# yoshitomo-matsubara/hnd-ghnd-object-detectors

Measured on AMD Instinct MI355X. Metric: distill-step images/sec at 3x800x1333, GHND Faster R-CNN b3ch, higher is better.
Workload: dtype f32

## Files before the change

hnd_ghnd_object_detectors_amd/_lib.py:

```python
import collections
import ctypes as C
import os
import re

_HERE = os.path.dirname(os.path.abspath(__file__))
LIB_PATH = os.environ.get('HND_LIB_PATH') or os.path.join(_HERE, 'libhnd_hip.so')
INCLUDE_DIR = os.path.join(os.path.dirname(_HERE), 'include')


class HndLibraryError(RuntimeError):
    pass


Header = collections.namedtuple('Header', 'defines enums structs functions')
_SCALARS = {'int': C.c_int, 'int32_t': C.c_int32, 'int64_t': C.c_int64, 'size_t': C.c_size_t, 'float': C.c_float,
            'double': C.c_double}
_POINTEES = ('void', 'float', 'double', 'int64_t', 'uint8_t', 'uint16_t', 'unsigned char')
_DIRECTIVE = re.compile(r'#\s*(include\s*<\w+\.h>|ifndef\s+\w+|define\s+\w+)$')
_TYPEDEF = re.compile(r'typedef\s+(enum|struct)\s+(\w+)\s*\{([^{}]*)\}\s*(\w+)\s*;')
_PROTOTYPE = re.compile(r'([^;{}()]+)\(([^;{}()]*)\)\s*;')
_DECLARATION = re.compile(r'\s*(?:const\s+)?(unsigned\s+char|\w+)(\s*\*+\s*|\s+)(\w+)\s*(\[\d*\])?\s*$')
_ENUMERATOR = re.compile(r'\s*(\w+)\s*=\s*(-?\d+)\s*$')
_SPACE = re.compile(r'\s*')

# ... 77 lines not shown
def _read(fname):
    path = os.path.join(INCLUDE_DIR, fname)
    if not os.path.isfile(path):
        raise HndLibraryError('C header %s not found: the binding of libhnd_hip.so is read from it' % path)
    with open(path) as f:
        return parse_header(f.read(), fname)


def _names(header, tag, prefix):
    if not all(k.startswith(prefix) for k in header.enums[tag]):
        raise HndLibraryError('enum %s: an enumerator without the prefix %s' % (tag, prefix))
    return {k[len(prefix):].lower(): v for k, v in header.enums[tag].items()}


HEADERS = {n: _read(n) for n in ('hnd_hip.h', 'hnd_optim.h', 'hnd_codec.h', 'hnd_qat.h')}
_HIP, _OPTIM, _CODEC, _QAT = HEADERS.values()

ConvDesc, WgradDesc, PackDesc, ImageDesc, BoxesDesc, MsePair, MimicPair = (
    _HIP.structs['hnd_' + n] for n in ('conv_desc', 'wgrad_desc', 'pack_desc', 'image_desc', 'boxes_desc', 'mse_pair', 'mimic_pair'))
OptimDesc = _OPTIM.structs['hnd_optim_desc']
MIMIC_KINDS = _names(_HIP, 'hnd_mimic_kind', 'HND_MIMIC_')
OPTIM_KINDS = _names(_OPTIM, 'hnd_optim_kind', 'HND_OPTIM_')
CONV_TILES = _names(_HIP, 'hnd_conv_tile', 'HND_TILE_')
WGRAD_VARIANTS = _names(_HIP, 'hnd_wgrad_variant', 'HND_WGRAD_')
ABI_VERSION, OPTIM_ABI = _HIP.defines['HND_ABI_VERSION'], _OPTIM.defines['HND_OPTIM_ABI']
CODEC_ABI, QAT_ABI = _CODEC.defines['HND_CODEC_ABI'], _QAT.defines['HND_QAT_ABI']
EXPORTED_SYMBOLS, OPTIM_SYMBOLS, CODEC_SYMBOLS, QAT_SYMBOLS = (tuple(sorted(h.functions)) for h in HEADERS.values())
QRANGE_HEADER_NAME = 'hnd_qrange.h'
QRANGE_HEADER = _read(QRANGE_HEADER_NAME)
QRANGE_ABI, QRANGE_SYMBOLS = QRANGE_HEADER.defines['HND_QRANGE_ABI'], tuple(sorted(QRANGE_HEADER.functions))
if QRANGE_HEADER.structs or QRANGE_HEADER.enums:
    raise HndLibraryError('%s declares a struct or an enum: it may declare functions only' % QRANGE_HEADER_NAME)

_lib = None


def load():
    global _lib
    if _lib is not None:
        return _lib
    if not os.path.exists(LIB_PATH):
        raise HndLibraryError(
            'libhnd_hip.so not found at %s: build it with `python -c "import __graft_entry__ as g; g.build()"` '
            '(or make -C hnd_ghnd_object_detectors_amd/csrc). There is no CPU fallback.' % LIB_PATH)
    import torch
    lib = C.CDLL(LIB_PATH)
    for header in list(HEADERS.values()) + [QRANGE_HEADER]:
        for name, (res, args) in header.functions.items():
            try:
                fn = getattr(lib, name)
            except AttributeError:
                raise HndLibraryError('libhnd_hip.so does not export %s (stale build?)' % name)
            fn.restype = res
            fn.argtypes = args
    if lib.hnd_abi_version() != ABI_VERSION:
        raise HndLibraryError('libhnd_hip.so ABI %d != expected %d' % (lib.hnd_abi_version(), ABI_VERSION))
    if lib.hnd_optim_abi() != OPTIM_ABI:
        raise HndLibraryError('libhnd_hip.so optimizer ABI %d != expected %d' % (lib.hnd_optim_abi(), OPTIM_ABI))
    if lib.hnd_codec_abi() != CODEC_ABI:
        raise HndLibraryError('libhnd_hip.so codec ABI %d != expected %d' % (lib.hnd_codec_abi(), CODEC_ABI))
    if lib.hnd_qat_abi() != QAT_ABI:
        raise HndLibraryError('libhnd_hip.so fake-quantisation ABI %d != expected %d' % (lib.hnd_qat_abi(), QAT_ABI))
    if lib.hnd_qrange_abi() != QRANGE_ABI:
        raise HndLibraryError('libhnd_hip.so quantisation-range ABI %d != expected %d' % (lib.hnd_qrange_abi(), QRANGE_ABI))
    _lib = lib
    return lib


def check(rc, what=''):
    if rc != 0:
        msg = load().hnd_last_error_string()
        raise RuntimeError('%s failed (status %d): %s' % (what or 'libhnd_hip call', rc,
                                                          msg.decode() if msg else '?'))
```

hnd_ghnd_object_detectors_amd/csrc/bf16x3.h:

```cpp
#pragma once
#include "common.h"

namespace hnd {

typedef __attribute__((ext_vector_type(8))) __bf16 bf8;
typedef __attribute__((ext_vector_type(4))) uint32_t u32x4;

__device__ __forceinline__ void split_pair(float x0, float x1, uint32_t& hp, uint32_t& mp, uint32_t& lp) {
  const uint32_t a0 = __float_as_uint(x0), a1 = __float_as_uint(x1);
  const uint32_t h0 = a0 & 0xffff0000u, h1 = a1 & 0xffff0000u;
  const float r0 = x0 - __uint_as_float(h0), r1 = x1 - __uint_as_float(h1);
  const uint32_t m0 = __float_as_uint(r0) & 0xffff0000u, m1 = __float_as_uint(r1) & 0xffff0000u;
  const float q0 = r0 - __uint_as_float(m0), q1 = r1 - __uint_as_float(m1);
  hp = __builtin_amdgcn_perm(h1, h0, 0x07060302u);
  mp = __builtin_amdgcn_perm(m1, m0, 0x07060302u);
  lp = __builtin_amdgcn_perm(__float_as_uint(q1), __float_as_uint(q0), 0x07060302u);
}

}
```

hnd_ghnd_object_detectors_amd/csrc/conv_bx3.hip:

```cpp

#include "bf16x3.h"
#include "common.h"

#include <stdlib.h>

namespace {

using hnd::bf8;
using hnd::cu_count;
using hnd::f32x4;
using hnd::FastDiv;
using hnd::split_pair;
using hnd::static_for;
using hnd::u32x4;

struct Bx3Args {
  FastDiv div_ow, div_oh;
  int nsl;
  int nchunks;
  int mrows;
  int cpg;
  int res_up;
};

template <int OFF>
__device__ __forceinline__ void rload(f32x4& dst, const float* p) {
  asm volatile("global_load_dwordx4 %0, %1, off offset:%2" : "=a"(dst) : "v"(p), "n"(OFF));
}
template <int CNT>
__device__ __forceinline__ void rwait(f32x4& a0, f32x4& a1, f32x4& a2, f32x4& a3, f32x4& a4, f32x4& a5, f32x4& a6,
                                      f32x4& a7) {
  asm volatile("s_waitcnt vmcnt(%8)"
               : "+a"(a0), "+a"(a1), "+a"(a2), "+a"(a3), "+a"(a4), "+a"(a5), "+a"(a6), "+a"(a7)
               : "n"(CNT));
}
// ... 211 lines not shown
            bwait8<32>(resm[2][0], resm[2][1], resm[2][2], resm[2][3], resm[3][0], resm[3][1], resm[3][2], resm[3][3]);
          }
        }
#pragma unroll
        for (int mi = 0; mi < MI; ++mi)
#pragma unroll
          for (int r = 0; r < 4; ++r) {
            const size_t m = (size_t)min(cc * 64 + mi * 16 + g4 * 4 + r, a.mrows - 1);
            f32x4 v;
#pragma unroll
            for (int ni = 0; ni < NI; ++ni) {
              float x = acc[mi][ni][r] * es[ni] + eb[ni];
              if (RES) x += resv[mi][r][ni];
              if (MK) x = ((resm[mi][r] >> ni) & 1u) ? x : 0.f;
              v[ni] = d.relu ? fmaxf(x, 0.f) : x;
            }
            const size_t yo = m * (size_t)d.ldc + col0;
            *(f32x4*)(d.y + yo) = v;
            if (MO)
              d.mask_out[yo >> 2] = (uint8_t)((v[0] > 0.f ? 1 : 0) | (v[1] > 0.f ? 2 : 0) | (v[2] > 0.f ? 4 : 0) |
                                              (v[3] > 0.f ? 8 : 0));
          }
#pragma unroll
        for (int mi = 0; mi < MI; ++mi) aptr[mi] = nptr[mi];
      }
      asm volatile("s_waitcnt vmcnt(0)" : "+v"(dummy)::"memory");
    }
    c = seg_hi;
  }
}

__global__ void pack_bx3_kernel(const float* __restrict__ w, uint16_t* __restrict__ img, int rows_pad, int K, int KI, int groups,
                                long long group_stride, long long total) {
  const int nsl = rows_pad / 64;
  const size_t plane = (size_t)64 * KI;
  for (long long e = blockIdx.x * (long long)blockDim.x + threadIdx.x; e < total; e += (long long)gridDim.x * blockDim.x) {
    const int k = (int)(e % K);
    long long t = e / K;
    const int row = (int)(t % rows_pad), g = (int)(t / rows_pad);
    const float x = w[(size_t)g * (size_t)group_stride + (size_t)row * K + k];
    const uint32_t xb = __float_as_uint(x), hb = xb & 0xffff0000u;
    const float r1 = x - __uint_as_float(hb);
    const uint32_t mb = __float_as_uint(r1) & 0xffff0000u;
    const float r2 = r1 - __uint_as_float(mb);
    const int part = k / KI, kk = k - part * KI;
    const int s = row / 64, r = row % 64, c = kk >> 3, pos = c ^ (r & 15);
    uint16_t* o = img + (((size_t)part * groups + g) * nsl + s) * 3 * plane + (size_t)r * KI + pos * 8 + (kk & 7);
    o[0] = (uint16_t)(hb >> 16);
    o[plane] = (uint16_t)(mb >> 16);
    o[2 * plane] = (uint16_t)(__float_as_uint(r2) >> 16);
  }
}

template <int KS, bool RES, bool MO, bool MK = false>
int launch_bx3_t(const hnd_conv_desc& d, const Bx3Args& a, int grid, hipStream_t stream) {
  const size_t lds = (size_t)3 * 64 * 32 * KS * sizeof(uint16_t);
  return hnd::launch_big_lds<bx3_kernel<KS, RES, MO, MK>>(dim3(grid), dim3(256), lds, 160 * 1024, stream, "hnd_conv2d_igemm(bx3)",
                                                          d, a);
}

}

namespace hnd {

static bool bx3_recommended(long long rows_per_image, int kdim, int cout) {
  if (rows_per_image <= 0 || cout <= 0 || cout % 64 != 0) return false;
  if (kdim != 128 && (kdim % 256 != 0 || kdim > 2048)) return false;
  const long long nteams = team_count(cout, 64);
  if (nteams == 0) return false;
  const long long chunks_at_16 = (rows_per_image * 16 + 63) / 64;
  return chunks_at_16 / nteams >= (kdim > 512 ? 16 : 8);
}

bool bx3_applies(const hnd_conv_desc& d) {
  if (!d.w_bf16x3) return false;
  if (d.kh != 1 || d.kw != 1 || d.bh != 0 || d.bw != 0 || d.cin != d.kdim) return false;
  if (d.kdim != 128 && (d.kdim % 256 != 0 || d.kdim > 2048)) return false;
  if (d.stats || d.pro_scale || d.res2 || d.mask || d.bwd_x) return false;
  if (d.mask_bits && d.mask_out) return false;
  if (d.mask_bits && d.kdim <= 256 && (!d.res1 || d.res1_mode != 0)) return false;
  if (d.res1 && ((uintptr_t)d.res1 % 16) != 0) return false;
  if (d.res1 && d.res1_mode == 1 && (d.yh != 2 * d.res1_h || d.yw != 2 * d.res1_w || d.ow % 4 != 0)) return false;
  if (d.cout % 64 != 0 || d.ldc % 4 != 0 || ((uintptr_t)d.y % 16) != 0) return false;
  if (team_count(d.cout, 64) == 0) return false;
// ... 61 lines not shown
  for (int p = 0; p < parts; ++p) {
    hnd_conv_desc q = d;
    if (p + 1 < parts) {
      q.relu = 0;
      q.mask_out = nullptr;
      q.mask_bits = nullptr;
    }
    if (p > 0) {
      q.x = d.x + (size_t)256 * p;
      q.w_bf16x3 = d.w_bf16x3 + part_elems * (size_t)p;
      q.epi_shift = nullptr;
      q.res1 = d.y;
      q.res1_mode = 0;
    }
    const int rc = launch_bx3_one(q, 256, stream);
    if (rc) return rc;
  }
  return 0;
}

}

extern "C" int hnd_bf16x3_recommended(int64_t rows_per_image, int kdim, int cout) {
  return hnd::bx3_recommended((long long)rows_per_image, kdim, cout) ? 1 : 0;
}

extern "C" size_t hnd_pack_bf16x3_elems(int rows_pad, int kdim, int groups) {
  if (rows_pad <= 0 || rows_pad % 64 != 0 || kdim <= 0 || kdim % 8 != 0 || groups < 1) return 0;
  return (size_t)groups * (size_t)rows_pad * (size_t)kdim * 3;
}

extern "C" int hnd_pack_bf16x3(const float* w_packed, uint16_t* img, int rows_pad, int kdim, int groups,
                               int64_t group_stride, void* stream) {
  HND_REQUIRE(w_packed && img && rows_pad > 0 && rows_pad % 64 == 0 && (kdim == 128 || (kdim % 256 == 0 && kdim <= 2048)) &&
                  groups >= 1 && (groups == 1 || group_stride >= (int64_t)rows_pad * kdim),
              "hnd_pack_bf16x3: bad arguments (kdim must be 128 or a multiple of 256 up to 2048)");
  const long long total = (long long)groups * rows_pad * kdim;
  long long blocks = (total + 255) / 256;
  if (blocks > 8192) blocks = 8192;
  hipLaunchKernelGGL(pack_bx3_kernel, dim3((unsigned)blocks), dim3(256), 0, hnd::as_stream(stream), w_packed, img, rows_pad,
                     kdim, kdim > 256 ? 256 : kdim, groups, (long long)group_stride, total);
  return hnd::check_launch("hnd_pack_bf16x3");
}
```

hnd_ghnd_object_detectors_amd/csrc/conv_bxs.hip:

```cpp

#include "bf16x3.h"
#include "common.h"
#include "conv_epilogue.h"
#include "stream_k_relay.h"

#include <stdlib.h>

namespace {

using hnd::bf8;
using hnd::f32x4;
using hnd::FastDiv;
using hnd::static_for;
using hnd::u32x4;

__device__ float g_bxs_zero_page[128];

struct BxsArgs {
  FastDiv div_ow, div_oh;
  FastDiv div_cin, div_kw;
  int mtiles, ntiles;
  int nit;
  int spin_limit;
  float* relay;
// ... 362 lines not shown
      hnd::epilogue_tile<MI, NI, true>(d, acc, rowoff, resoff, 4 * g4, col0, es, eb, s1, s2, full);
      if (d.stats) {
        const int cl = wn * 64 + l16 * 4;
#pragma unroll
        for (int ni = 0; ni < NI; ++ni) {
          float a1 = s1[ni], a2 = s2[ni];
          a1 += __shfl_xor(a1, 16); a2 += __shfl_xor(a2, 16);
          a1 += __shfl_xor(a1, 32); a2 += __shfl_xor(a2, 32);
          if (g4 == 0) {
            red[(wm * 2 + 0) * BN + cl + ni] = a1;
            red[(wm * 2 + 1) * BN + cl + ni] = a2;
          }
        }
        asm volatile("s_waitcnt lgkmcnt(0)\n\ts_barrier" ::: "memory");
        for (int e = tid; e < (WM / 2) * BN; e += 256) {
          const int half = e / BN, c = e - half * BN;
          const long long st_tile = (long long)mt * (WM / 2) + half;
          if (st_tile * 128 < M) {
            float* st = d.stats + (size_t)st_tile * 2 * d.cout + nt * BN + c;
            st[0] = red[((2 * half) * 2 + 0) * BN + c] + red[((2 * half + 1) * 2 + 0) * BN + c];
            st[d.cout] = red[((2 * half) * 2 + 1) * BN + c] + red[((2 * half + 1) * 2 + 1) * BN + c];
          }
        }
        asm volatile("s_waitcnt lgkmcnt(0)\n\ts_barrier" ::: "memory");
      }
    }
  }
  asm volatile("s_waitcnt vmcnt(0)" ::: "memory");
  launch_done();
}

__global__ void pack_bxs_kernel(const float* __restrict__ w, uint16_t* __restrict__ img, int rows_pad, int K, int groups,
                                long long group_stride, long long total) {
  const int nsl = rows_pad / 64, nst = K / 64;
  for (long long e = blockIdx.x * (long long)blockDim.x + threadIdx.x; e < total; e += (long long)gridDim.x * blockDim.x) {
    const int k = (int)(e % K);
    long long t = e / K;
    const int row = (int)(t % rows_pad), g = (int)(t / rows_pad);
    const float x = w[(size_t)g * (size_t)group_stride + (size_t)row * K + k];
    const uint32_t xb = __float_as_uint(x), hb = xb & 0xffff0000u;
    const float r1 = x - __uint_as_float(hb);
    const uint32_t mb = __float_as_uint(r1) & 0xffff0000u;
    const float r2 = r1 - __uint_as_float(mb);
    const int s = row / 64, r = row % 64, st = k / 64, kk = k % 64, c = kk >> 3, pos = c ^ ((r >> 1) & 7);
    uint16_t* o = img + ((((size_t)g * nsl + s) * nst + st) * 3) * 4096 + (size_t)r * 64 + pos * 8 + (kk & 7);
    o[0] = (uint16_t)(hb >> 16);
    o[4096] = (uint16_t)(mb >> 16);
    o[8192] = (uint16_t)(__float_as_uint(r2) >> 16);
  }
}

template <int WN, bool PRO, bool TAPS>
int launch_t(const hnd_conv_desc& d, const BxsArgs& a, size_t lds, int grid, hipStream_t stream) {
  return hnd::launch_big_lds<bxs_kernel<WN, PRO, TAPS>>(dim3(grid), dim3(256), lds, 160 * 1024, stream, "hnd_conv2d_igemm(bxs)",
                                                        d, a);
}

template <int WN>
int launch_w(const hnd_conv_desc& d, const BxsArgs& a, size_t lds, int grid, hipStream_t stream) {
  const bool taps = hnd::has_taps(d);
  if (d.pro_scale) return taps ? launch_t<WN, true, true>(d, a, lds, grid, stream)
                               : launch_t<WN, true, false>(d, a, lds, grid, stream);
  return taps ? launch_t<WN, false, true>(d, a, lds, grid, stream) : launch_t<WN, false, false>(d, a, lds, grid, stream);
}

size_t bxs_lds_bytes(const hnd_conv_desc& d, int wn) {
  return (size_t)(wn == 1 ? 2 : 3) * 2 * 3 * 4096 * sizeof(uint16_t) + (d.pro_scale ? 2 * (size_t)d.cin : 0) * sizeof(float) +
         4 * 128 * sizeof(int) + (size_t)(4 / wn) * 2 * 64 * wn * sizeof(float);
}

}

namespace hnd {

int bxs_variant(const hnd_conv_desc& d) {
  if (!d.w_bf16x3s) return 0;
  if (d.cin % 64 != 0 || d.kdim % 128 != 0 || d.kdim < 128) return 0;
  const bool taps = has_taps(d);
  if (taps ? (d.kdim != d.kh * d.kw * d.cin) : (d.kdim != d.cin)) return 0;
  if (!taps && !samples_inside(d)) return 0;
  if (d.cout % 64 != 0 || d.cout > 4096 || d.cin > 4096) return 0;
  if ((long long)d.n * d.h * d.w_ * d.cin >= (1ll << 32)) return 0;
// ... 6 lines not shown
}

int launch_bxs(const hnd_conv_desc& d, int wn, hipStream_t stream) {
  BxsArgs a;
  int grid;
  if (const int rc = relay_launch_check("bxs", a.spin_limit, a.err)) return rc;
  a.div_ow = make_fastdiv((unsigned)d.ow);
  a.div_oh = make_fastdiv((unsigned)d.oh);
  a.div_cin = make_fastdiv((unsigned)d.cin);
  a.div_kw = make_fastdiv((unsigned)d.kw);
  relay_grid(d, wn, a.mtiles, a.ntiles, grid);
  a.nit = d.kdim / 128;
  a.relay = (d.relay_ws && relay_workspace(d, wn) > 0) ? d.relay_ws : nullptr;
  const size_t lds = bxs_lds_bytes(d, wn);
  return wn == 2 ? launch_w<2>(d, a, lds, grid, stream) : launch_w<1>(d, a, lds, grid, stream);
}

}

extern "C" int hnd_bf16x3s_recommended(int64_t rows_per_image, int kdim, int cout, int taps) {
  (void)taps;
  if (rows_per_image <= 0 || cout <= 0 || cout % 64 != 0 || kdim % 128 != 0) return 0;
  if (hnd::env_begins_with_0("HND_BXS")) return 0;
  return (rows_per_image * 16 >= 16384 && kdim >= 256) ? 1 : 0;
}

extern "C" size_t hnd_pack_bf16x3s_elems(int rows_pad, int kdim, int groups) {
  if (rows_pad <= 0 || rows_pad % 64 != 0 || kdim <= 0 || kdim % 128 != 0 || groups < 1) return 0;
  return (size_t)groups * (size_t)rows_pad * (size_t)kdim * 3;
}

extern "C" int hnd_pack_bf16x3s(const float* w_packed, uint16_t* img, int rows_pad, int kdim, int groups, int64_t group_stride,
                                void* stream) {
  HND_REQUIRE(w_packed && img && rows_pad > 0 && rows_pad % 64 == 0 && kdim > 0 && kdim % 128 == 0 && groups >= 1 &&
                  (groups == 1 || group_stride >= (int64_t)rows_pad * kdim),
              "hnd_pack_bf16x3s: bad arguments (rows_pad %% 64, kdim %% 128)");
  const long long total = (long long)groups * rows_pad * kdim;
  long long blocks = (total + 255) / 256;
  if (blocks > 8192) blocks = 8192;
  hipLaunchKernelGGL(pack_bxs_kernel, dim3((unsigned)blocks), dim3(256), 0, hnd::as_stream(stream), w_packed, img, rows_pad,
                     kdim, groups, (long long)group_stride, total);
  return hnd::check_launch("hnd_pack_bf16x3s");
}
```

hnd_ghnd_object_detectors_amd/csrc/elementwise.hip:

```cpp
#include "common.h"
#include "hnd_codec.h"
#include "hnd_qat.h"
#include "hnd_qrange.h"

#include <hip/hip_fp16.h>
#include <float.h>
#include <limits.h>
#include <math.h>
#include <cmath>

namespace {

using hnd::f32x4;

constexpr int kMaxBlocks = 256 * 16;

inline int grid_for(long long work_items, int threads = 256) {
  long long b = (work_items + threads - 1) / threads;
  if (b < 1) b = 1;
  if (b > kMaxBlocks) b = kMaxBlocks;
  return (int)b;
}

constexpr int kEwU = 4;
// ... 264 lines not shown
    f32x4 r;                                                                     \
    r.x = (a).x > 0.f ? (g).x * s.x : 0.f; r.y = (a).y > 0.f ? (g).y * s.y : 0.f; \
    r.z = (a).z > 0.f ? (g).z * s.z : 0.f; r.w = (a).w > 0.f ? (g).w * s.w : 0.f; \
    *(f32x4*)(dx + (xo)) = r;                                                    \
  }
    f32x4 g = z4;
    HND_TAKE(g, i00, d00, 4)
    HND_PUT(x00, a00, g)
    if (col1) {
      g = z4;
      HND_TAKE(g, i00, d00, 5)
      HND_TAKE(g, i01, d01, 3)
      HND_PUT(x01, a01, g)
    }
    if (row1) {
      g = z4;
      HND_TAKE(g, i00, d00, 7)
      HND_TAKE(g, i10, d10, 1)
      HND_PUT(x10, a10, g)
    }
    if (row1 && col1) {
      g = z4;
      HND_TAKE(g, i00, d00, 8)
      HND_TAKE(g, i01, d01, 6)
      HND_TAKE(g, i10, d10, 2)
      HND_TAKE(g, i11, d11, 0)
      HND_PUT(x11, a11, g)
    }
#undef HND_TAKE
#undef HND_PUT
  }
}

__global__ void __launch_bounds__(1024) bn_finalize_kernel(const float* __restrict__ partials, int ntiles, int c, int cs,
                                   double count, const float* gamma, const float* beta, float* running_mean,
                                   float* running_var, long long* nbt, float momentum, float eps, float* scale,
                                   float* shift, float* save_mean, float* save_rstd) {
  __shared__ double red[2][16][16];
  const int lane = threadIdx.x & 63, wave = threadIdx.x >> 6;
  const int cl = lane & 15, ts = lane >> 4;
  const int ch = blockIdx.x * 16 + cl;
  double s1 = 0.0, s2 = 0.0;
  if (ch < c) {
    int t = wave * 4 + ts;
    for (; t + 3 * 64 < ntiles; t += 4 * 64) {
      float a[4], b[4];
#pragma unroll
      for (int u = 0; u < 4; ++u) {
        a[u] = partials[((size_t)(t + u * 64) * 2 + 0) * cs + ch];
        b[u] = partials[((size_t)(t + u * 64) * 2 + 1) * cs + ch];
      }
#pragma unroll
      for (int u = 0; u < 4; ++u) { s1 += (double)a[u]; s2 += (double)b[u]; }
    }
    for (; t < ntiles; t += 64) {
      s1 += (double)partials[((size_t)t * 2 + 0) * cs + ch];
      s2 += (double)partials[((size_t)t * 2 + 1) * cs + ch];
    }
  }
  s1 += __shfl_xor(s1, 16); s2 += __shfl_xor(s2, 16);
  s1 += __shfl_xor(s1, 32); s2 += __shfl_xor(s2, 32);
  if (ts == 0) { red[0][wave][cl] = s1; red[1][wave][cl] = s2; }
  __syncthreads();
  if (threadIdx.x >= 16 || ch >= cs) return;
  if (ch >= c) {
    scale[ch] = 0.f; shift[ch] = 0.f; save_mean[ch] = 0.f; save_rstd[ch] = 0.f;
// ... 93 lines not shown
      const long long p = pb + (long long)rows * u;
      if (p < p1) {
        const size_t o = (size_t)p * cs + c4 * 4;
        dv[u] = HND_NT_LOAD4(g + o);
        xq[u] = HND_NT_LOAD4(x + o);
      }
    }
#pragma unroll
    for (int u = 0; u < kEwU; ++u) {
      if (pb + (long long)rows * u >= p1) continue;
      f32x4 d = dv[u];
      const f32x4 xv = xq[u];
      if (relu) {
        const f32x4 out = xv * sc + sh;
        d.x = out.x > 0.f ? d.x : 0.f; d.y = out.y > 0.f ? d.y : 0.f;
        d.z = out.z > 0.f ? d.z : 0.f; d.w = out.w > 0.f ? d.w : 0.f;
      }
      s1 += d;
      s2 += d * ((xv - mu) * rs);
    }
  }
#pragma unroll
  for (int k = 0; k < 4; ++k) { red[0][threadIdx.x][k] = s1[k]; red[1][threadIdx.x][k] = s2[k]; }
  __syncthreads();
  for (int idx = threadIdx.x; idx < cs * 2; idx += 256) {
    const int which = idx / cs, ch = idx - which * cs;
    const int g4 = ch >> 2, k = ch & 3;
    float s = 0.f;
    for (int rr = 0; rr < rows; ++rr) s += red[which][rr * cs4 + g4][k];
    partials[((size_t)blockIdx.x * 2 + which) * cs + ch] = s;
  }
}

__global__ void bn_bwd_finalize_kernel(const float* __restrict__ partials, int ntiles, int c, int cs, double count,
                                       const float* gamma, const float* mean, const float* rstd, float* dgamma,
                                       float* dbeta, float* k123) {
  const int lane = threadIdx.x & 63;
  const int ch = blockIdx.x * (blockDim.x >> 6) + (threadIdx.x >> 6);
  if (ch >= cs) return;
  if (ch >= c) {
    if (lane == 0) { k123[ch] = 0.f; k123[cs + ch] = 0.f; k123[2 * cs + ch] = 0.f; }
    return;
  }
  double s1 = 0.0, s2 = 0.0;
  for (int t = lane; t < ntiles; t += 64) {
    s1 += (double)partials[((size_t)t * 2 + 0) * cs + ch];
    s2 += (double)partials[((size_t)t * 2 + 1) * cs + ch];
  }
  s1 = wave_sum_d(s1);
  s2 = wave_sum_d(s2);
  if (lane == 0) {
    dbeta[ch] = (float)s1;
    dgamma[ch] = (float)s2;
    const double k1 = (double)gamma[ch] * (double)rstd[ch];
    const double k2 = -k1 * (double)rstd[ch] * s2 / count;
    const double k3 = k1 * ((double)mean[ch] * (double)rstd[ch] * s2 - s1) / count;
    k123[ch] = (float)k1;
    k123[cs + ch] = (float)k2;
    k123[2 * cs + ch] = (float)k3;
  }
}

__global__ void bn_bwd_apply_kernel(const float* __restrict__ g, const float* __restrict__ x,
                                    const float* __restrict__ scale, const float* __restrict__ shift,
                                    const float* __restrict__ k123, int relu, float* __restrict__ dx, long long n4,
                                    int cs) {
  const int cs4 = cs >> 2;
  const bool fixed = (256 % cs4) == 0;
  int c4 = threadIdx.x % cs4;
  f32x4 sc = *(const f32x4*)(scale + c4 * 4), sh = *(const f32x4*)(shift + c4 * 4);
  f32x4 k1 = *(const f32x4*)(k123 + c4 * 4), k2 = *(const f32x4*)(k123 + cs + c4 * 4),
        k3 = *(const f32x4*)(k123 + 2 * cs + c4 * 4);
  const long long chunk = 256ll * kEwU;
  for (long long base = blockIdx.x * chunk + threadIdx.x; base < n4; base += (long long)gridDim.x * chunk) {
    f32x4 dv[kEwU], xv[kEwU];
#pragma unroll
    for (int u = 0; u < kEwU; ++u) {
      const long long e = base + 256ll * u;
      if (e < n4) {
        dv[u] = HND_NT_LOAD4(g + e * 4);
        xv[u] = HND_NT_LOAD4(x + e * 4);
// ... 960 lines not shown

int hnd_affine_relu(const float* x, const float* scale, const float* shift, float* y, int64_t npix, int cs, int relu,
                    uint8_t* mask_out, void* stream) {
  HND_REQUIRE(x && scale && shift && y && npix > 0 && cs > 0 && cs % 4 == 0, "hnd_affine_relu: bad arguments");
  const long long n4 = (long long)npix * (cs / 4);
  hipLaunchKernelGGL(affine_relu_kernel, dim3(grid_for_chunks(n4)), dim3(256), 0, hnd::as_stream(stream), x, scale,
                     shift, y, n4, cs / 4, relu, mask_out);
  return hnd::check_launch("hnd_affine_relu");
}

int hnd_relu_mask_nibbles(const float* x, uint8_t* bits, int64_t n4, void* stream) {
  HND_REQUIRE(x && bits && n4 > 0 && ((uintptr_t)x % 16) == 0, "hnd_relu_mask_nibbles: bad arguments");
  hipLaunchKernelGGL(relu_mask_nibbles_kernel, dim3(grid_for_chunks(n4)), dim3(256), 0, hnd::as_stream(stream), x, bits,
                     (long long)n4);
  return hnd::check_launch("hnd_relu_mask_nibbles");
}

int hnd_bn_bwd_ntiles(int64_t npix) { return (int)((npix + kBnTilePix - 1) / kBnTilePix); }

int hnd_bn_bwd_reduce(const float* g, const float* x, const float* scale, const float* shift, const float* mean,
                      const float* rstd, int relu, int64_t npix, int cs, float* partials, void* stream) {
  HND_REQUIRE(g && x && scale && shift && mean && rstd && partials, "hnd_bn_bwd_reduce: null pointer");
  HND_REQUIRE(npix > 0 && cs % 4 == 0 && cs <= 1024 && 256 % (cs / 4) == 0,
              "hnd_bn_bwd_reduce: channel stride %d must be 4*2^k <= 1024", cs);
  hipLaunchKernelGGL(bn_bwd_reduce_kernel, dim3(hnd_bn_bwd_ntiles(npix)), dim3(256), 0, hnd::as_stream(stream), g, x,
                     scale, shift, mean, rstd, relu, (long long)npix, cs, partials);
  return hnd::check_launch("hnd_bn_bwd_reduce");
}

int hnd_bn_bwd_finalize(const float* partials, int ntiles, int c, int cs, int64_t count, const float* gamma,
                        const float* mean, const float* rstd, float* dgamma, float* dbeta, float* k123, void* stream) {
  HND_REQUIRE(partials && gamma && mean && rstd && dgamma && dbeta && k123, "hnd_bn_bwd_finalize: null pointer");
  HND_REQUIRE(ntiles > 0 && c > 0 && cs >= c && count > 0, "hnd_bn_bwd_finalize: bad sizes");
  hipLaunchKernelGGL(bn_bwd_finalize_kernel, dim3((cs + 3) / 4), dim3(256), 0, hnd::as_stream(stream), partials, ntiles,
                     c, cs, (double)count, gamma, mean, rstd, dgamma, dbeta, k123);
  return hnd::check_launch("hnd_bn_bwd_finalize");
}

int hnd_bn_bwd_apply(const float* g, const float* x, const float* scale, const float* shift, const float* k123,
                     int relu, float* dx, int64_t npix, int cs, void* stream) {
  HND_REQUIRE(g && x && scale && shift && k123 && dx && npix > 0 && cs % 4 == 0, "hnd_bn_bwd_apply: bad arguments");
  const long long n4 = (long long)npix * (cs / 4);
  hipLaunchKernelGGL(bn_bwd_apply_kernel, dim3(grid_for_chunks(n4)), dim3(256), 0, hnd::as_stream(stream), g, x, scale,
                     shift, k123, relu, dx, n4, cs);
  return hnd::check_launch("hnd_bn_bwd_apply");
}

size_t hnd_mse_scratch_elems(void) { return (size_t)kMseBlocks * kMaxPairs; }

int hnd_mse_sum_fwd_bwd(const hnd_mse_pair* pairs, int npairs, double* loss_out, double* scratch, void* stream) {
  HND_REQUIRE(pairs && loss_out && scratch, "hnd_mse_sum_fwd_bwd: null pointer");
  HND_REQUIRE(npairs >= 1 && npairs <= kMaxPairs, "hnd_mse_sum_fwd_bwd: 1..%d pairs supported", kMaxPairs);
  MseArgs a;
  a.npairs = npairs;
  long long total = 0;
  for (int k = 0; k < npairs; ++k) {
    HND_REQUIRE(pairs[k].teacher && pairs[k].student && pairs[k].numel > 0 && pairs[k].numel % 4 == 0,
                "hnd_mse_sum_fwd_bwd: pair %d invalid (numel must be a positive multiple of 4)", k);
    a.pair[k] = pairs[k];
    total += pairs[k].numel;
  }
  const int used = loss_split_blocks(pairs, npairs, total, a.first_block);
  hipStream_t s = hnd::as_stream(stream);
  hipLaunchKernelGGL(mse_kernel, dim3(used), dim3(256), 0, s, a, scratch);
  int rc = hnd::check_launch("hnd_mse_sum_fwd_bwd");
  if (rc) return rc;
  hipLaunchKernelGGL(mse_finalize_kernel, dim3(1), dim3(64 * kMaxPairs), 0, s, a, scratch, loss_out);
// ... 373 lines not shown
```

hnd_ghnd_object_detectors_amd/ops.py:

```python
import ctypes as C
import os
import math

import torch

from . import _lib
from ._lib import ConvDesc, WgradDesc, MsePair, MimicPair, MIMIC_KINDS, check

_L = _lib.load()
TILE_NAMES = {code: name for name, code in _lib.CONV_TILES.items()}
WGRAD_NAMES = {code: name for name, code in _lib.WGRAD_VARIANTS.items()}
PARAM_EPOCH = [0]


def stream_ptr():
    return torch.cuda.current_stream().cuda_stream


def ptr(t):
    return None if t is None else t.data_ptr()


def round_up(x, m):
    return (x + m - 1) // m * m
# ... 53 lines not shown
          'hnd_pack_bf16x3')
    return out


def bxs_image(buf, rows_pad, kdim, groups=1, group_stride=0, out=None, force=None):
    if out is None:
        out = torch.empty(int(_L.hnd_pack_bf16x3s_elems(rows_pad, kdim, groups)), dtype=torch.int16, device=buf.device)
    check(_L.hnd_pack_bf16x3s(buf.data_ptr(), out.data_ptr(), rows_pad, kdim, groups, int(group_stride), stream_ptr()),
          'hnd_pack_bf16x3s')
    return out


class PackedWeight(object):
    groups, group_stride, taps, bx3, bxs = 1, 0, 1, None, None

    def __init__(self, buf, rows, kdim, chan_pad, chan_real=None, groups=1, group_stride=0, taps=1):
        self.buf, self.rows, self.rows_pad, self.kdim = buf, rows, round_up(rows, 64), kdim
        self.chan_pad, self.chan_real = chan_pad, chan_pad if chan_real is None else chan_real
        self.groups, self.group_stride, self.taps = groups, group_stride, taps
        self.bx3 = self.bxs = None

    def fill(self):
        """(re)compute buf from the source weight (nothing to do for a buffer the caller filled)"""

    def repack(self):
        self.fill()
        self.refresh_images()

    def refresh_images(self):
        if self.bx3 is not None:
            bx3_image(self.buf, self.rows_pad, self.kdim, self.groups, self.group_stride, out=self.bx3)
        if self.bxs is not None:
            bxs_image(self.buf, self.rows_pad, self.kdim, self.groups, self.group_stride, out=self.bxs)

    def can_bx3(self):
        return (self.taps == 1 and self.kdim == self.chan_pad and self.rows_pad % 64 == 0
                and (self.kdim == 128 or (self.kdim % 256 == 0 and self.kdim <= 2048)))

    def can_bxs(self):
        return (self.groups == 1 and self.kdim % 128 == 0 and self.chan_pad % 64 == 0 and self.rows_pad % 64 == 0
                and self.kdim == self.taps * self.chan_pad)

    def attach(self, which):
        if which == 'bx3':
            if self.bx3 is None and self.can_bx3():
                self.bx3 = bx3_image(self.buf, self.rows_pad, self.kdim, self.groups, self.group_stride)
            return self.bx3
        if self.bxs is None and self.can_bxs():
            self.bxs = bxs_image(self.buf, self.rows_pad, self.kdim, self.groups, self.group_stride)
        return self.bxs


class DirectWeights(PackedWeight):
    def __init__(self, w, transposed=False, chan_pad=None, taps=None, kscale=None):
        cout, cin, kh, kw = w.shape
        assert w.is_contiguous() and w.dtype == torch.float32
        if taps is None:
            taps = (0, 1, kh, 0, 1, kw)
        i0, istep, ni, j0, jstep, nj = taps
        chans = cout if transposed else cin
        rows = cin if transposed else cout
        if chan_pad is None:
            chan_pad = chan_pad_of(chans)
        kdim = round_up(ni * nj * chan_pad, 32)
        PackedWeight.__init__(self, torch.empty(round_up(rows, 64) * kdim, dtype=torch.float32, device=w.device), rows,
                              kdim, chan_pad, chans, taps=ni * nj)
        self.src, self.kscale = w, kscale
        self.args = (cout, cin, kh, kw, int(transposed), chan_pad, i0, istep, ni, j0, jstep, nj)
        self.repack()

    def repack(self):
        if PACK_BATCH['open'] and self.kscale is None:
            PACK_BATCH['items'].append(self)
        else:
            PackedWeight.repack(self)

    def fill(self):
        check(_L.hnd_pack_weights(self.src.data_ptr(), self.buf.data_ptr(), *self.args, stream_ptr()), 'hnd_pack_weights')
        if self.kscale is not None:
            check(_L.hnd_scale_packed_k(self.buf.data_ptr(), self.rows_pad, self.kdim, self.taps, self.chan_pad,
                                        self.kscale.data_ptr(), min(self.kscale.numel(), self.chan_pad), stream_ptr()),
                  'hnd_scale_packed_k')


pack_weights = DirectWeights


PACK_BATCH = {'open': False, 'items': []}


def pack_batch_begin():
    PACK_BATCH['open'], PACK_BATCH['items'] = True, []


def pack_batch_end():
    from ._lib import PackDesc
    items, PACK_BATCH['open'], PACK_BATCH['items'] = PACK_BATCH['items'], False, []
    if not items:
        return
    arr = (PackDesc * len(items))()
    for d, pw in zip(arr, items):
        d.src, d.dst = pw.src.data_ptr(), pw.buf.data_ptr()
        (d.cout, d.cin, d.kh, d.kw, d.transposed, d.chan_pad, d.i0, d.istep, d.ni, d.j0, d.jstep, d.nj) = pw.args
    check(_L.hnd_pack_weights_batched(arr, len(items), stream_ptr()), 'hnd_pack_weights_batched')
    for pw in items:
        pw.refresh_images()


def fbn_fold(weight, bias, mean, var, eps=0.0, cs=None, out=None):
    c = weight.numel()
    cs = cs or c
    if out is not None:
        scale, shift = out
        assert scale.numel() == cs and shift.numel() == cs
    else:
        scale = torch.empty(cs, dtype=torch.float32, device=weight.device)
        shift = torch.empty(cs, dtype=torch.float32, device=weight.device)
    check(_L.hnd_fbn_fold(ptr(weight), ptr(bias), ptr(mean), ptr(var), ptr(scale), ptr(shift), c, cs, float(eps),
                          stream_ptr()), 'hnd_fbn_fold')
    return scale, shift


class ConvLaunch(object):
    __slots__ = ('desc', 'ref', 'keep', 'flops', 'alg_flops', 'variant', 'build', 'relay')

    def __init__(self, desc, keep, flops=0):
        self.desc, self.keep, self.flops = desc, keep, flops
        self.alg_flops = flops
        self.ref = C.byref(desc)
        self.relay = None
        self.refresh_variant()

    def refresh_variant(self):
        need = int(_L.hnd_conv2d_igemm_workspace(self.ref))
        if need == 0:
            self.relay, self.desc.relay_ws = None, None
        elif self.relay is None or self.relay.numel() * 4 < need:
            self.relay = torch.zeros((need + 3) // 4, dtype=torch.float32, device=torch.device('cuda', torch.cuda.current_device()))
            self.desc.relay_ws = self.relay.data_ptr()
# ... 573 lines not shown
    _qrange_bits(who, bits)
    _qrange_geometry(who, x, c)
    _qrange_qparams(who, qparams)
    if x.dim() != 4:
        raise ValueError('%s: x must be [N, H, W, cs]' % who)
    n, h, w, cs = x.shape
    if not (payload.dtype == torch.uint8 and payload.is_contiguous()
            and payload.numel() == codec_packed_bytes(n * c * h * w, bits) > 0):
        raise ValueError('%s: payload must be %d uint8 bytes' % (who, codec_packed_bytes(n * c * h * w, bits)))
    check(_L.hnd_quantize_pack_range_bits(ptr(x), n, h, w, c, cs, bits, ptr(payload), ptr(qparams), stream_ptr()),
          'hnd_quantize_pack_range_bits')


def roundtrip_f16(x):
    check(_L.hnd_roundtrip_f16(ptr(x), x.numel(), stream_ptr()), 'hnd_roundtrip_f16')


def wino_tiles_pad(n, h, w, tile=2):
    return int(_L.hnd_wino_tiles_pad(n, h, w, tile))


class _WinogradWeights(PackedWeight):
    def __init__(self, weight, dgrad, tile):
        cout, cin, kh, kw = weight.shape
        assert kh == self.K and kw == self.K and weight.is_contiguous() and tile in self.TILES
        rows, depth = (cin, cout) if dgrad else (cout, cin)
        assert depth % 32 == 0, 'Winograd path needs a GEMM depth that is a multiple of 32'
        ncomp, rows_pad = (tile + self.K - 1) ** 2, round_up(rows, 64)
        PackedWeight.__init__(self, torch.empty(ncomp * rows_pad * depth, dtype=torch.float32, device=weight.device),
                              rows, depth, depth, groups=ncomp, group_stride=rows_pad * depth)
        self.src, self.dgrad, self.tile, self.ncomp, self.depth = weight, dgrad, tile, ncomp, depth
        self.repack()

    def fill(self):
        check(getattr(_L, self.KERNEL)(ptr(self.src), ptr(self.buf), self.src.shape[0], self.src.shape[1],
                                       int(self.dgrad), self.tile, stream_ptr()), self.KERNEL)


class WinoWeights(_WinogradWeights):
    K, TILES, KERNEL = 3, (2, 4, 6), 'hnd_wino_weights'

    def __init__(self, weight, dgrad=False, tile=2):
        _WinogradWeights.__init__(self, weight, dgrad, tile)


def _component_gemms(v, ww, m, cout, tiles_pad, n, oh, ow):
    tiles = ((oh + ww.tile - 1) // ww.tile) * ((ow + ww.tile - 1) // ww.tile)
    gemm = conv_desc(v, ww, m, kh=1, kw=1, oh=1, ow=ww.ncomp * tiles_pad, sh=1, dh=1, bh=0, sw=1, dw=1, bw=0, cout=cout,
                     rows_per_image=ww.ncomp * tiles, w_group_rows=tiles_pad)
    gemm.flops = 2 * ww.ncomp * n * tiles * ww.rows * ww.depth
    gemm.alg_flops = 2 * n * oh * ow * ww.rows * ww.K ** 2 * ww.depth
    return gemm


class WinoConv(object):

    def __init__(self, x, ww, y, v, m, pro_scale=None, pro_shift=None, pro_relu=False, epi_scale=None, epi_shift=None,
                 res1=None, mask=None, relu=False, mask_out=None):
        n, h, w, c = _nhwc(x)
        assert tuple(y.shape[:3]) == (n, h, w) and c == ww.depth
        self.x, self.y, self.ww = x, y, ww
        self.geom = (n, h, w, c)
        tile, nc = ww.tile, ww.ncomp
        self.tile = tile
        self.tiles_pad = wino_tiles_pad(n, h, w, tile)
        self.cout = round_up(ww.rows, 4)
# ... 345 lines not shown
```

Measured before the change: 215.2.

## Batch bf16x3 weight-image packing into one launch and widen BN backward finalize

Per-weight bf16x3 and bf16x3s image packing launches after each optimizer step are gathered into a single batched kernel, with up to 32 images per launch and a block-offset table. Winograd weights join the batch when it is open, which cuts per-kernel launch and Python overhead during the repack phase. Separately, the BN backward finalize kernel now uses 1024-thread blocks over 16 channels, with unrolled strided loads reduced through shared memory, to give more memory parallelism on the partial-sum reduction. The risk is that the batch kernel finds its item with a linear search per block, and the shared-memory reduction changes the order of the double-precision summation.

```diff
diff --git a/hnd_ghnd_object_detectors_amd/_lib.py b/hnd_ghnd_object_detectors_amd/_lib.py
--- a/hnd_ghnd_object_detectors_amd/_lib.py
+++ b/hnd_ghnd_object_detectors_amd/_lib.py
@@ -133,6 +133,12 @@
 if QRANGE_HEADER.structs or QRANGE_HEADER.enums:
     raise HndLibraryError('%s declares a struct or an enum: it may declare functions only' % QRANGE_HEADER_NAME)
 
+PACKIMG_HEADER_NAME = 'hnd_packimg.h'
+PACKIMG_HEADER = _read(PACKIMG_HEADER_NAME)
+PACKIMG_ABI, PACKIMG_SYMBOLS = PACKIMG_HEADER.defines['HND_PACKIMG_ABI'], tuple(sorted(PACKIMG_HEADER.functions))
+ImagePackDesc = PACKIMG_HEADER.structs['hnd_image_pack_desc']
+IMAGE_KINDS = _names(PACKIMG_HEADER, 'hnd_image_kind', 'HND_IMAGE_')
+
 _lib = None
 
 
@@ -146,7 +152,7 @@
             '(or make -C hnd_ghnd_object_detectors_amd/csrc). There is no CPU fallback.' % LIB_PATH)
     import torch
     lib = C.CDLL(LIB_PATH)
-    for header in list(HEADERS.values()) + [QRANGE_HEADER]:
+    for header in list(HEADERS.values()) + [QRANGE_HEADER, PACKIMG_HEADER]:
         for name, (res, args) in header.functions.items():
             try:
                 fn = getattr(lib, name)
@@ -164,6 +170,8 @@
         raise HndLibraryError('libhnd_hip.so fake-quantisation ABI %d != expected %d' % (lib.hnd_qat_abi(), QAT_ABI))
     if lib.hnd_qrange_abi() != QRANGE_ABI:
         raise HndLibraryError('libhnd_hip.so quantisation-range ABI %d != expected %d' % (lib.hnd_qrange_abi(), QRANGE_ABI))
+    if lib.hnd_packimg_abi() != PACKIMG_ABI:
+        raise HndLibraryError('libhnd_hip.so image-pack ABI %d != expected %d' % (lib.hnd_packimg_abi(), PACKIMG_ABI))
     _lib = lib
     return lib
 
diff --git a/hnd_ghnd_object_detectors_amd/csrc/bf16x3.h b/hnd_ghnd_object_detectors_amd/csrc/bf16x3.h
--- a/hnd_ghnd_object_detectors_amd/csrc/bf16x3.h
+++ b/hnd_ghnd_object_detectors_amd/csrc/bf16x3.h
@@ -17,4 +17,61 @@
   lp = __builtin_amdgcn_perm(__float_as_uint(q1), __float_as_uint(q0), 0x07060302u);
 }
 
+
+__device__ __forceinline__ void pack_bx3_body(const float* __restrict__ w, uint16_t* __restrict__ img, int rows_pad, int K,
+                                              int KI, int groups, long long group_stride, long long total, int block,
+                                              int nblocks) {
+  const int nsl = rows_pad / 64;
+  const size_t plane = (size_t)64 * KI;
+  for (long long e = block * (long long)blockDim.x + threadIdx.x; e < total; e += (long long)nblocks * blockDim.x) {
+    const int k = (int)(e % K);
+    long long t = e / K;
+    const int row = (int)(t % rows_pad), g = (int)(t / rows_pad);
+    const float x = w[(size_t)g * (size_t)group_stride + (size_t)row * K + k];
+    const uint32_t xb = __float_as_uint(x), hb = xb & 0xffff0000u;
+    const float r1 = x - __uint_as_float(hb);
+    const uint32_t mb = __float_as_uint(r1) & 0xffff0000u;
+    const float r2 = r1 - __uint_as_float(mb);
+    const int part = k / KI, kk = k - part * KI;
+    const int s = row / 64, r = row % 64, c = kk >> 3, pos = c ^ (r & 15);
+    uint16_t* o = img + (((size_t)part * groups + g) * nsl + s) * 3 * plane + (size_t)r * KI + pos * 8 + (kk & 7);
+    o[0] = (uint16_t)(hb >> 16);
+    o[plane] = (uint16_t)(mb >> 16);
+    o[2 * plane] = (uint16_t)(__float_as_uint(r2) >> 16);
+  }
 }
+
+__device__ __forceinline__ void pack_bxs_body(const float* __restrict__ w, uint16_t* __restrict__ img, int rows_pad, int K,
+                                              int groups, long long group_stride, long long total, int block, int nblocks) {
+  const int nsl = rows_pad / 64, nst = K / 64;
+  for (long long e = block * (long long)blockDim.x + threadIdx.x; e < total; e += (long long)nblocks * blockDim.x) {
+    const int k = (int)(e % K);
+    long long t = e / K;
+    const int row = (int)(t % rows_pad), g = (int)(t / rows_pad);
+    const float x = w[(size_t)g * (size_t)group_stride + (size_t)row * K + k];
+    const uint32_t xb = __float_as_uint(x), hb = xb & 0xffff0000u;
+    const float r1 = x - __uint_as_float(hb);
+    const uint32_t mb = __float_as_uint(r1) & 0xffff0000u;
+    const float r2 = r1 - __uint_as_float(mb);
+    const int s = row / 64, r = row % 64, st = k / 64, kk = k % 64, c = kk >> 3, pos = c ^ ((r >> 1) & 7);
+    uint16_t* o = img + ((((size_t)g * nsl + s) * nst + st) * 3) * 4096 + (size_t)r * 64 + pos * 8 + (kk & 7);
+    o[0] = (uint16_t)(hb >> 16);
+    o[4096] = (uint16_t)(mb >> 16);
+    o[8192] = (uint16_t)(__float_as_uint(r2) >> 16);
+  }
+}
+
+inline bool pack_bx3_args_ok(const float* w, const uint16_t* img, int rows_pad, int kdim, int groups, int64_t group_stride) {
+  return w && img && rows_pad > 0 && rows_pad % 64 == 0 && (kdim == 128 || (kdim % 256 == 0 && kdim <= 2048)) && groups >= 1 &&
+         (groups == 1 || group_stride >= (int64_t)rows_pad * kdim);
+}
+inline bool pack_bxs_args_ok(const float* w, const uint16_t* img, int rows_pad, int kdim, int groups, int64_t group_stride) {
+  return w && img && rows_pad > 0 && rows_pad % 64 == 0 && kdim > 0 && kdim % 128 == 0 && groups >= 1 &&
+         (groups == 1 || group_stride >= (int64_t)rows_pad * kdim);
+}
+inline int pack_image_blocks(long long total) {
+  long long blocks = (total + 255) / 256;
+  return (int)(blocks > 8192 ? 8192 : blocks);
+}
+
+}
diff --git a/hnd_ghnd_object_detectors_amd/csrc/conv_bx3.hip b/hnd_ghnd_object_detectors_amd/csrc/conv_bx3.hip
--- a/hnd_ghnd_object_detectors_amd/csrc/conv_bx3.hip
+++ b/hnd_ghnd_object_detectors_amd/csrc/conv_bx3.hip
@@ -1,6 +1,7 @@
 
 #include "bf16x3.h"
 #include "common.h"
+#include "hnd_packimg.h"
 
 #include <stdlib.h>
 
@@ -278,24 +279,27 @@
 
 __global__ void pack_bx3_kernel(const float* __restrict__ w, uint16_t* __restrict__ img, int rows_pad, int K, int KI, int groups,
                                 long long group_stride, long long total) {
-  const int nsl = rows_pad / 64;
-  const size_t plane = (size_t)64 * KI;
-  for (long long e = blockIdx.x * (long long)blockDim.x + threadIdx.x; e < total; e += (long long)gridDim.x * blockDim.x) {
-    const int k = (int)(e % K);
-    long long t = e / K;
-    const int row = (int)(t % rows_pad), g = (int)(t / rows_pad);
-    const float x = w[(size_t)g * (size_t)group_stride + (size_t)row * K + k];
-    const uint32_t xb = __float_as_uint(x), hb = xb & 0xffff0000u;
-    const float r1 = x - __uint_as_float(hb);
-    const uint32_t mb = __float_as_uint(r1) & 0xffff0000u;
-    const float r2 = r1 - __uint_as_float(mb);
-    const int part = k / KI, kk = k - part * KI;
-    const int s = row / 64, r = row % 64, c = kk >> 3, pos = c ^ (r & 15);
-    uint16_t* o = img + (((size_t)part * groups + g) * nsl + s) * 3 * plane + (size_t)r * KI + pos * 8 + (kk & 7);
-    o[0] = (uint16_t)(hb >> 16);
-    o[plane] = (uint16_t)(mb >> 16);
-    o[2 * plane] = (uint16_t)(__float_as_uint(r2) >> 16);
-  }
+  hnd::pack_bx3_body(w, img, rows_pad, K, KI, groups, group_stride, total, blockIdx.x, gridDim.x);
+}
+
+constexpr int kMaxBatchImages = 32;
+struct ImageBatch {
+  const float* w[kMaxBatchImages];
+  uint16_t* img[kMaxBatchImages];
+  long long group_stride[kMaxBatchImages], total[kMaxBatchImages];
+  int rows_pad[kMaxBatchImages], K[kMaxBatchImages], groups[kMaxBatchImages], kind[kMaxBatchImages];
+  int first[kMaxBatchImages + 1];
+  int n;
+};
+__global__ void pack_images_batch_kernel(const ImageBatch b) {
+  int i = 0;
+  while (i + 1 < b.n && (int)blockIdx.x >= b.first[i + 1]) ++i;
+  const int block = (int)blockIdx.x - b.first[i], nblocks = b.first[i + 1] - b.first[i];
+  if (b.kind[i] == HND_IMAGE_BXS)
+    hnd::pack_bxs_body(b.w[i], b.img[i], b.rows_pad[i], b.K[i], b.groups[i], b.group_stride[i], b.total[i], block, nblocks);
+  else
+    hnd::pack_bx3_body(b.w[i], b.img[i], b.rows_pad[i], b.K[i], b.K[i] > 256 ? 256 : b.K[i], b.groups[i], b.group_stride[i],
+                       b.total[i], block, nblocks);
 }
 
 template <int KS, bool RES, bool MO, bool MK = false>
@@ -423,13 +427,52 @@
 
 extern "C" int hnd_pack_bf16x3(const float* w_packed, uint16_t* img, int rows_pad, int kdim, int groups,
                                int64_t group_stride, void* stream) {
-  HND_REQUIRE(w_packed && img && rows_pad > 0 && rows_pad % 64 == 0 && (kdim == 128 || (kdim % 256 == 0 && kdim <= 2048)) &&
-                  groups >= 1 && (groups == 1 || group_stride >= (int64_t)rows_pad * kdim),
+  HND_REQUIRE(hnd::pack_bx3_args_ok(w_packed, img, rows_pad, kdim, groups, group_stride),
               "hnd_pack_bf16x3: bad arguments (kdim must be 128 or a multiple of 256 up to 2048)");
   const long long total = (long long)groups * rows_pad * kdim;
-  long long blocks = (total + 255) / 256;
-  if (blocks > 8192) blocks = 8192;
+  const int blocks = hnd::pack_image_blocks(total);
   hipLaunchKernelGGL(pack_bx3_kernel, dim3((unsigned)blocks), dim3(256), 0, hnd::as_stream(stream), w_packed, img, rows_pad,
                      kdim, kdim > 256 ? 256 : kdim, groups, (long long)group_stride, total);
   return hnd::check_launch("hnd_pack_bf16x3");
 }
+
+extern "C" int hnd_packimg_abi(void) { return HND_PACKIMG_ABI; }
+
+extern "C" int hnd_pack_images_capacity(void) { return kMaxBatchImages; }
+
+extern "C" int hnd_pack_images_batched(const hnd_image_pack_desc* descs, int n, void* stream) {
+  HND_REQUIRE(n >= 0 && (descs || n == 0), "hnd_pack_images_batched: bad arguments");
+  for (int i = 0; i < n; ++i) {
+    const hnd_image_pack_desc& d = descs[i];
+    HND_REQUIRE(d.kind == HND_IMAGE_BX3 || d.kind == HND_IMAGE_BXS, "hnd_pack_images_batched: item %d: unknown kind %d", i,
+                d.kind);
+    HND_REQUIRE(d.kind == HND_IMAGE_BXS ? hnd::pack_bxs_args_ok(d.src, d.img, d.rows_pad, d.kdim, d.groups, d.group_stride)
+                                        : hnd::pack_bx3_args_ok(d.src, d.img, d.rows_pad, d.kdim, d.groups, d.group_stride),
+                "hnd_pack_images_batched: item %d: bad arguments (those of hnd_pack_bf16x3 / hnd_pack_bf16x3s)", i);
+  }
+  for (int i0 = 0; i0 < n; i0 += kMaxBatchImages) {
+    ImageBatch b;
+    b.n = n - i0 < kMaxBatchImages ? n - i0 : kMaxBatchImages;
+    b.first[0] = 0;
+    for (int k = 0; k < b.n; ++k) {
+      const hnd_image_pack_desc& d = descs[i0 + k];
+      b.w[k] = d.src;
+      b.img[k] = d.img;
+      b.group_stride[k] = (long long)d.group_stride;
+      b.total[k] = (long long)d.groups * d.rows_pad * d.kdim;
+      b.rows_pad[k] = d.rows_pad;
+      b.K[k] = d.kdim;
+      b.groups[k] = d.groups;
+      b.kind[k] = d.kind;
+      b.first[k + 1] = b.first[k] + hnd::pack_image_blocks(b.total[k]);
+    }
+    for (int k = b.n; k < kMaxBatchImages; ++k) {
+      b.w[k] = nullptr; b.img[k] = nullptr; b.group_stride[k] = 0; b.total[k] = 0;
+      b.rows_pad[k] = 0; b.K[k] = 0; b.groups[k] = 0; b.kind[k] = 0; b.first[k + 1] = b.first[b.n];
+    }
+    hipLaunchKernelGGL(pack_images_batch_kernel, dim3((unsigned)b.first[b.n]), dim3(256), 0, hnd::as_stream(stream), b);
+    const int rc = hnd::check_launch("hnd_pack_images_batched");
+    if (rc) return rc;
+  }
+  return 0;
+}
diff --git a/hnd_ghnd_object_detectors_amd/csrc/conv_bxs.hip b/hnd_ghnd_object_detectors_amd/csrc/conv_bxs.hip
--- a/hnd_ghnd_object_detectors_amd/csrc/conv_bxs.hip
+++ b/hnd_ghnd_object_detectors_amd/csrc/conv_bxs.hip
@@ -418,22 +418,7 @@
 
 __global__ void pack_bxs_kernel(const float* __restrict__ w, uint16_t* __restrict__ img, int rows_pad, int K, int groups,
                                 long long group_stride, long long total) {
-  const int nsl = rows_pad / 64, nst = K / 64;
-  for (long long e = blockIdx.x * (long long)blockDim.x + threadIdx.x; e < total; e += (long long)gridDim.x * blockDim.x) {
-    const int k = (int)(e % K);
-    long long t = e / K;
-    const int row = (int)(t % rows_pad), g = (int)(t / rows_pad);
-    const float x = w[(size_t)g * (size_t)group_stride + (size_t)row * K + k];
-    const uint32_t xb = __float_as_uint(x), hb = xb & 0xffff0000u;
-    const float r1 = x - __uint_as_float(hb);
-    const uint32_t mb = __float_as_uint(r1) & 0xffff0000u;
-    const float r2 = r1 - __uint_as_float(mb);
-    const int s = row / 64, r = row % 64, st = k / 64, kk = k % 64, c = kk >> 3, pos = c ^ ((r >> 1) & 7);
-    uint16_t* o = img + ((((size_t)g * nsl + s) * nst + st) * 3) * 4096 + (size_t)r * 64 + pos * 8 + (kk & 7);
-    o[0] = (uint16_t)(hb >> 16);
-    o[4096] = (uint16_t)(mb >> 16);
-    o[8192] = (uint16_t)(__float_as_uint(r2) >> 16);
-  }
+  hnd::pack_bxs_body(w, img, rows_pad, K, groups, group_stride, total, blockIdx.x, gridDim.x);
 }
 
 template <int WN, bool PRO, bool TAPS>
@@ -506,12 +491,10 @@
 
 extern "C" int hnd_pack_bf16x3s(const float* w_packed, uint16_t* img, int rows_pad, int kdim, int groups, int64_t group_stride,
                                 void* stream) {
-  HND_REQUIRE(w_packed && img && rows_pad > 0 && rows_pad % 64 == 0 && kdim > 0 && kdim % 128 == 0 && groups >= 1 &&
-                  (groups == 1 || group_stride >= (int64_t)rows_pad * kdim),
+  HND_REQUIRE(hnd::pack_bxs_args_ok(w_packed, img, rows_pad, kdim, groups, group_stride),
               "hnd_pack_bf16x3s: bad arguments (rows_pad %% 64, kdim %% 128)");
   const long long total = (long long)groups * rows_pad * kdim;
-  long long blocks = (total + 255) / 256;
-  if (blocks > 8192) blocks = 8192;
+  const int blocks = hnd::pack_image_blocks(total);
   hipLaunchKernelGGL(pack_bxs_kernel, dim3((unsigned)blocks), dim3(256), 0, hnd::as_stream(stream), w_packed, img, rows_pad,
                      kdim, groups, (long long)group_stride, total);
   return hnd::check_launch("hnd_pack_bf16x3s");
diff --git a/hnd_ghnd_object_detectors_amd/csrc/elementwise.hip b/hnd_ghnd_object_detectors_amd/csrc/elementwise.hip
--- a/hnd_ghnd_object_detectors_amd/csrc/elementwise.hip
+++ b/hnd_ghnd_object_detectors_amd/csrc/elementwise.hip
@@ -320,6 +320,35 @@
   }
 }
 
+constexpr int kBnChainU = 16;
+__device__ __forceinline__ void bn_chain_sums(const float* __restrict__ partials, int ntiles, int cs, int ch, int t0,
+                                              double& s1, double& s2) {
+  int t = t0;
+  for (; t + (kBnChainU - 1) * 64 < ntiles; t += kBnChainU * 64) {
+    float a[kBnChainU], b[kBnChainU];
+#pragma unroll
+    for (int u = 0; u < kBnChainU; ++u) {
+      a[u] = partials[((size_t)(t + u * 64) * 2 + 0) * cs + ch];
+      b[u] = partials[((size_t)(t + u * 64) * 2 + 1) * cs + ch];
+    }
+#pragma unroll
+    for (int u = 0; u < kBnChainU; ++u) { s1 += (double)a[u]; s2 += (double)b[u]; }
+  }
+  if (t < ntiles) {
+    float a[kBnChainU - 1], b[kBnChainU - 1];
+#pragma unroll
+    for (int u = 0; u < kBnChainU - 1; ++u) {
+      const bool in = t + u * 64 < ntiles;
+      const size_t tt = in ? (size_t)(t + u * 64) : (size_t)t;
+      a[u] = partials[(tt * 2 + 0) * cs + ch];
+      b[u] = partials[(tt * 2 + 1) * cs + ch];
+    }
+#pragma unroll
+    for (int u = 0; u < kBnChainU - 1; ++u)
+      if (t + u * 64 < ntiles) { s1 += (double)a[u]; s2 += (double)b[u]; }
+  }
+}
+
 __global__ void __launch_bounds__(1024) bn_finalize_kernel(const float* __restrict__ partials, int ntiles, int c, int cs,
                                    double count, const float* gamma, const float* beta, float* running_mean,
                                    float* running_var, long long* nbt, float momentum, float eps, float* scale,
@@ -479,21 +508,27 @@
   }
 }
 
-__global__ void bn_bwd_finalize_kernel(const float* __restrict__ partials, int ntiles, int c, int cs, double count,
-                                       const float* gamma, const float* mean, const float* rstd, float* dgamma,
-                                       float* dbeta, float* k123) {
-  const int lane = threadIdx.x & 63;
-  const int ch = blockIdx.x * (blockDim.x >> 6) + (threadIdx.x >> 6);
+__global__ void __launch_bounds__(1024) bn_bwd_finalize_kernel(const float* __restrict__ partials, int ntiles, int c, int cs,
+                                       double count, const float* gamma, const float* mean, const float* rstd,
+                                       float* dgamma, float* dbeta, float* k123) {
+  __shared__ double red[2][16][65];
+  const int lane = threadIdx.x & 63, wave = threadIdx.x >> 6;
+  {
+    const int cl = lane & 15, ts = lane >> 4;
+    const int chl = blockIdx.x * 16 + cl;
+    double c1 = 0.0, c2 = 0.0;
+    if (chl < c) bn_chain_sums(partials, ntiles, cs, chl, wave * 4 + ts, c1, c2);
+    red[0][cl][wave * 4 + ts] = c1;
+    red[1][cl][wave * 4 + ts] = c2;
+  }
+  __syncthreads();
+  const int ch = blockIdx.x * 16 + wave;
   if (ch >= cs) return;
   if (ch >= c) {
     if (lane == 0) { k123[ch] = 0.f; k123[cs + ch] = 0.f; k123[2 * cs + ch] = 0.f; }
     return;
   }
-  double s1 = 0.0, s2 = 0.0;
-  for (int t = lane; t < ntiles; t += 64) {
-    s1 += (double)partials[((size_t)t * 2 + 0) * cs + ch];
-    s2 += (double)partials[((size_t)t * 2 + 1) * cs + ch];
-  }
+  double s1 = red[0][wave][lane], s2 = red[1][wave][lane];
   s1 = wave_sum_d(s1);
   s2 = wave_sum_d(s2);
   if (lane == 0) {
@@ -1520,7 +1555,7 @@
                         const float* mean, const float* rstd, float* dgamma, float* dbeta, float* k123, void* stream) {
   HND_REQUIRE(partials && gamma && mean && rstd && dgamma && dbeta && k123, "hnd_bn_bwd_finalize: null pointer");
   HND_REQUIRE(ntiles > 0 && c > 0 && cs >= c && count > 0, "hnd_bn_bwd_finalize: bad sizes");
-  hipLaunchKernelGGL(bn_bwd_finalize_kernel, dim3((cs + 3) / 4), dim3(256), 0, hnd::as_stream(stream), partials, ntiles,
+  hipLaunchKernelGGL(bn_bwd_finalize_kernel, dim3((cs + 15) / 16), dim3(1024), 0, hnd::as_stream(stream), partials, ntiles,
                      c, cs, (double)count, gamma, mean, rstd, dgamma, dbeta, k123);
   return hnd::check_launch("hnd_bn_bwd_finalize");
 }
diff --git a/hnd_ghnd_object_detectors_amd/ops.py b/hnd_ghnd_object_detectors_amd/ops.py
--- a/hnd_ghnd_object_detectors_amd/ops.py
+++ b/hnd_ghnd_object_detectors_amd/ops.py
@@ -109,6 +109,9 @@
             bx3_image(self.buf, self.rows_pad, self.kdim, self.groups, self.group_stride, out=self.bx3)
         if self.bxs is not None:
             bxs_image(self.buf, self.rows_pad, self.kdim, self.groups, self.group_stride, out=self.bxs)
+
+    def image_items(self):
+        return [(kind, img) for kind, img in (('bx3', self.bx3), ('bxs', self.bxs)) if img is not None]
 
     def can_bx3(self):
         return (self.taps == 1 and self.kdim == self.chan_pad and self.rows_pad % 64 == 0
@@ -163,25 +166,36 @@
 pack_weights = DirectWeights
 
 
-PACK_BATCH = {'open': False, 'items': []}
+PACK_BATCH = {'open': False, 'items': [], 'filled': []}
 
 
 def pack_batch_begin():
-    PACK_BATCH['open'], PACK_BATCH['items'] = True, []
+    PACK_BATCH['open'], PACK_BATCH['items'], PACK_BATCH['filled'] = True, [], []
 
 
 def pack_batch_end():
     from ._lib import PackDesc
-    items, PACK_BATCH['open'], PACK_BATCH['items'] = PACK_BATCH['items'], False, []
-    if not items:
-        return
-    arr = (PackDesc * len(items))()
-    for d, pw in zip(arr, items):
-        d.src, d.dst = pw.src.data_ptr(), pw.buf.data_ptr()
-        (d.cout, d.cin, d.kh, d.kw, d.transposed, d.chan_pad, d.i0, d.istep, d.ni, d.j0, d.jstep, d.nj) = pw.args
-    check(_L.hnd_pack_weights_batched(arr, len(items), stream_ptr()), 'hnd_pack_weights_batched')
-    for pw in items:
-        pw.refresh_images()
+    items, filled = PACK_BATCH['items'], PACK_BATCH['filled']
+    PACK_BATCH['open'], PACK_BATCH['items'], PACK_BATCH['filled'] = False, [], []
+    if items:
+        arr = (PackDesc * len(items))()
+        for d, pw in zip(arr, items):
+            d.src, d.dst = pw.src.data_ptr(), pw.buf.data_ptr()
+            (d.cout, d.cin, d.kh, d.kw, d.transposed, d.chan_pad, d.i0, d.istep, d.ni, d.j0, d.jstep, d.nj) = pw.args
+        check(_L.hnd_pack_weights_batched(arr, len(items), stream_ptr()), 'hnd_pack_weights_batched')
+    pack_images_batched(items + filled)
+
+
+def pack_images_batched(operands):
+    todo = [(pw, kind, img) for pw in operands for kind, img in pw.image_items()]
+    if not todo:
+        return 0
+    arr = (_lib.ImagePackDesc * len(todo))()
+    for d, (pw, kind, img) in zip(arr, todo):
+        d.src, d.img, d.kind = pw.buf.data_ptr(), img.data_ptr(), _lib.IMAGE_KINDS[kind]
+        d.rows_pad, d.kdim, d.groups, d.group_stride = pw.rows_pad, pw.kdim, pw.groups, int(pw.group_stride)
+    check(_L.hnd_pack_images_batched(arr, len(todo), stream_ptr()), 'hnd_pack_images_batched')
+    return len(todo)
 
 
 def fbn_fold(weight, bias, mean, var, eps=0.0, cs=None, out=None):
@@ -821,6 +835,13 @@
         self.src, self.dgrad, self.tile, self.ncomp, self.depth = weight, dgrad, tile, ncomp, depth
         self.repack()
 
+    def repack(self):
+        if PACK_BATCH['open']:
+            self.fill()
+            PACK_BATCH['filled'].append(self)
+        else:
+            PackedWeight.repack(self)
+
     def fill(self):
         check(getattr(_L, self.KERNEL)(ptr(self.src), ptr(self.buf), self.src.shape[0], self.src.shape[1],
                                        int(self.dgrad), self.tile, stream_ptr()), self.KERNEL)
diff --git a/include/hnd_packimg.h b/include/hnd_packimg.h
--- /dev/null
+++ b/include/hnd_packimg.h
@@ -0,0 +1,33 @@
+#ifndef HND_PACKIMG_H
+#define HND_PACKIMG_H
+
+#include <stddef.h>
+#include <stdint.h>
+
+#ifdef __cplusplus
+extern "C" {
+#endif
+
+#define HND_PACKIMG_ABI 1
+
+typedef enum hnd_image_kind {
+  HND_IMAGE_BX3 = 0,
+  HND_IMAGE_BXS = 1
+} hnd_image_kind;
+
+typedef struct hnd_image_pack_desc {
+  const float* src;
+  uint16_t* img;
+  int32_t kind;
+  int32_t rows_pad, kdim, groups;
+  int64_t group_stride;
+} hnd_image_pack_desc;
+
+int hnd_packimg_abi(void);
+int hnd_pack_images_capacity(void);
+int hnd_pack_images_batched(const hnd_image_pack_desc* descs, int n, void* stream);
+
+#ifdef __cplusplus
+}
+#endif
+#endif
```

New measurement: 216.7 (median of 3 runs). About the same (+0.7%).
